# wfus/Fully-Homomorphic-Image-Processing

Measured on AMD Instinct MI355X. Metric: encrypted 8x8 blocks/sec (homomorphic DCT+quant), higher is better.
Workload: dtype f64

## Files before the change

### fully-homomorphic-image-processing_amd/csrc/dct_fused.hip

```cpp
#include "internal.h"

#include <cstdlib>

#include "fp64_core.h"

#pragma clang fp contract(off)

namespace {
using namespace fp64;

template <int L, int LE> struct Shape {
    static constexpr int N = 1 << L, E = 1 << LE, TP = N >> LE, NP = (L + LE - 1) / LE, LDS_WORDS = N + (N >> LE);
};
__host__ __device__ constexpr int g_lo(int L, int LE, int p) { return (L - LE * p - LE) < 0 ? 0 : (L - LE * p - LE); }
__host__ __device__ constexpr int g_stages(int L, int LE, int p) { return (L - LE * p) > LE ? LE : (L - LE * p); }
template <int LO, int LE> __device__ __forceinline__ int g_index(int tid, int r) {
    return ((tid >> LO) << (LO + LE)) | (r << LO) | (tid & ((1 << LO) - 1));
}
template <int LO, int LE> __device__ __forceinline__ int g_pad(int j) { return j + ((j >> (LO + LE)) << LO); }

template <int L, int LE, int P> struct PassTw {
    static constexpr int LO = g_lo(L, LE, P), S = g_stages(L, LE, P), NTW = (1 << LE) - 1;
    static constexpr int rb(int u) { return (L - 1 - (LE * P + u)) - LO; }
    static constexpr int count(int u) { return 1 << (LE - 1 - rb(u)); }
// ... 70 lines not shown
            for (int b0 = 0; b0 < E / 2; b0 += KB) {
                double t[KB * M], wm[KB * M];
#pragma unroll
                for (int kb = 0; kb < KB; kb++) {
                    const int b = b0 + kb, r0 = ((b >> rb) << (rb + 1)) | (b & ((1 << rb) - 1)), r1 = r0 | (1 << rb);
                    const double wv = w[T::offset(u) + (r0 >> (rb + 1))];
#pragma unroll
                    for (int m = 0; m < M; m++) {
                        const double X = x[m][r0], Y = x[m][r1];
                        x[m][r0] = X + Y;
                        t[kb * M + m] = X - Y; wm[kb * M + m] = wv;
                    }
                }
                mmv<KB * M>(t, wm, p, pinv);
#pragma unroll
                for (int kb = 0; kb < KB; kb++) {
                    const int b = b0 + kb, r0 = ((b >> rb) << (rb + 1)) | (b & ((1 << rb) - 1)), r1 = r0 | (1 << rb);
#pragma unroll
                    for (int m = 0; m < M; m++) x[m][r1] = t[kb * M + m];
                }
            }
        }
    }
}

template <int L, int LE, int LO_FROM, int LO_TO, int M>
__device__ __forceinline__ void transpose(double (&x)[M][1 << LE], double *lds, int tid, int &phase) {
    constexpr int PL = imin(LO_FROM, LO_TO), E = 1 << LE;
    constexpr bool WAVE_LOCAL = (Shape<L, LE>::TP <= 64) || (LO_FROM <= 6 && LO_TO <= 6);
#pragma unroll
    for (int m = 0; m < M; m++) {
        double *buf = lds + (phase & 1) * Shape<L, LE>::LDS_WORDS;
        phase++;
#pragma unroll
        for (int r = 0; r < E; r++) buf[g_pad<PL, LE>(g_index<LO_FROM, LE>(tid, r))] = x[m][r];
        if constexpr (WAVE_LOCAL) {
            __builtin_amdgcn_fence(__ATOMIC_RELEASE, "wavefront");
            __builtin_amdgcn_wave_barrier();
            __builtin_amdgcn_fence(__ATOMIC_ACQUIRE, "wavefront");
        } else {
            __syncthreads();
        }
#pragma unroll
        for (int r = 0; r < E; r++) x[m][r] = buf[g_pad<PL, LE>(g_index<LO_TO, LE>(tid, r))];
    }
}

template <int L, int LE, int M, typename PRE, int P = 0>
__device__ __forceinline__ void ntt_fwd(double (&x)[M][1 << LE], double (&w)[(1 << LE) - 1], const double *__restrict__ tw, double p, double pinv,
                                        double *lds, int tid, int &phase, PRE pre) {
    if constexpr (P + 1 < Shape<L, LE>::NP) {
        double wn[(1 << LE) - 1];
        if (LE >= 4) load_tw<L, LE, P + 1>(wn, tw, tid);
        fwd_pass<L, LE, P, M>(x, w, p, pinv);
        if (LE < 4) load_tw<L, LE, P + 1>(wn, tw, tid);
        if constexpr (P + 2 == Shape<L, LE>::NP) pre();
        transpose<L, LE, g_lo(L, LE, P), g_lo(L, LE, P + 1), M>(x, lds, tid, phase);
        ntt_fwd<L, LE, M, PRE, P + 1>(x, wn, tw, p, pinv, lds, tid, phase, pre);
    } else {
        fwd_pass<L, LE, P, M>(x, w, p, pinv);
    }
}
template <int L, int LE, int M, bool BIG, int P = Shape<L, LE>::NP - 1>
__device__ __forceinline__ void ntt_inv(double (&x)[M][1 << LE], double (&w)[(1 << LE) - 1], const double *__restrict__ itw, double p, double pinv,
                                        double *lds, int tid, int &phase) {
    if constexpr (P > 0) {
        double wn[(1 << LE) - 1];
        if (LE >= 4) load_tw<L, LE, P - 1>(wn, itw, tid);
        inv_pass<L, LE, P, M>(x, w, 0.0, p, pinv);
        if (LE < 4) load_tw<L, LE, P - 1>(wn, itw, tid);
        if constexpr (BIG) {
#pragma unroll
            for (int m = 0; m < M; m++)
#pragma unroll
                for (int r = 0; r < (1 << LE); r++) x[m][r] = red(x[m][r], p, pinv);
        }
        transpose<L, LE, g_lo(L, LE, P), g_lo(L, LE, P - 1), M>(x, lds, tid, phase);
        ntt_inv<L, LE, M, BIG, P - 1>(x, wn, itw, p, pinv, lds, tid, phase);
    } else {
        inv_pass<L, LE, P, M>(x, w, itw[0], p, pinv);
    }
}

constexpr double PACK_BIAS = 6755399441055744.0;
template <int E, int TP>
__device__ __forceinline__ void store_packed(char *__restrict__ ob, u32 vo, u32 so, const double (&x)[E]) {
    static_assert(E == 8, "packed layout is defined for 8 values per thread");
    u32 lo[8], hi[8];
#pragma unroll
    for (int r = 0; r < 8; r++) {
        const double t = x[r] + PACK_BIAS;
        lo[r] = (u32)__double2loint(t);
        hi[r] = (u32)__double2hiint(t);
    }
#pragma unroll
    for (int q = 0; q < 4; q++) *(u64 *)(ob + (size_t)(so + q * TP * 8) + vo) = (u64)lo[2 * q] | ((u64)lo[2 * q + 1] << 32);
    u32 h[2];
#pragma unroll
    for (int g = 0; g < 2; g++) {
        const u32 p01 = __builtin_amdgcn_perm(hi[4 * g + 1], hi[4 * g + 0], 0x0c0c0400u);
        const u32 p23 = __builtin_amdgcn_perm(hi[4 * g + 3], hi[4 * g + 2], 0x0c0c0400u);
        h[g] = __builtin_amdgcn_perm(p23, p01, 0x05040100u);
    }
    *(u64 *)(ob + (size_t)(so + 4 * TP * 8) + vo) = (u64)h[0] | ((u64)h[1] << 32);
}
typedef __attribute__((address_space(3))) void lc_lptr;
template <int NT>
__device__ __forceinline__ void stage_consts(gwin_t w, u32 voff, u32 soff, u32 cstride_bytes, double *stg) {
#pragma unroll
    for (int i0 = 0; i0 < NT; i0 += 2) {
        const int i = (i0 + 1 < NT) ? i0 : NT - 2;
        __builtin_amdgcn_raw_ptr_buffer_load_lds(w, (lc_lptr *)(stg + i * 64), 16, voff, soff + (u32)i * cstride_bytes, 0, 0);
    }
}

template <int L, int LE, bool BIG, int HALF, bool PACK, bool LDSC>
__device__ __forceinline__ void rows_body(const u64 *__restrict__ in, double *__restrict__ mid, const double *__restrict__ consts,
                                          const double *__restrict__ tw, const Work &wk, double p, double pinv, u32 k, double *lds) {
    using SH = Shape<L, LE>;
    constexpr int N = SH::N, TP = SH::TP, E = SH::E, NC = HalfC<HALF>::NC, FIRST = HalfC<HALF>::FIRST;
    const int tid = threadIdx.x;
    const size_t poly_words = (size_t)k * N, ct_words = 2 * poly_words;
    const size_t base = ((size_t)wk.blk * 64 + 8 * wk.line) * ct_words + (size_t)wk.poly * poly_words + (size_t)wk.prime * N;
    const gwin_t win_in = gwin(in + base), win_mid = gwin(mid + base);
    const u32 vo = (u32)tid * 8u, ctb = (u32)(ct_words * 8);
    double w0[E - 1];
    load_tw<L, LE, 0>(w0, tw, tid);
    double x[4][E];
    u64 ra[2][E], rb[2][E];
    auto issue = [&](int m) {
#pragma unroll
        for (int r = 0; r < E; r++) {
            ra[m & 1][r] = gld_u64(win_in, vo, (u32)m * ctb + r * TP * 8);
            rb[m & 1][r] = gld_u64(win_in, vo, (u32)(7 - m) * ctb + r * TP * 8);
        }
    };
    auto combine = [&](int m) {
#pragma unroll
        for (int r = 0; r < E; r++) {
            const u64 A = ra[m & 1][r], B = rb[m & 1][r];
            x[m][r] = HALF ? u52_biased(A) - u52_biased(B) : u52_to_f64(A + B);
        }
    };
    if constexpr (LE >= 4) {
        issue(0);
        issue(1);
        asm volatile("" ::: "memory");
        combine(0);
        issue(2);
        asm volatile("" ::: "memory");
        combine(1);
        issue(3);
        asm volatile("" ::: "memory");
        combine(2);
        combine(3);
    } else {
#pragma unroll
        for (int m = 0; m < 4; m++) {
            issue(m);
            combine(m);
            asm volatile("" ::: "memory");
        }
    }
    const size_t cstride = (size_t)k * N;
    const gwin_t win_c = gwin(consts + (size_t)FIRST * cstride + (size_t)wk.prime * N);
    const u32 csb = (u32)(cstride * 8);
    double cn[9];
    auto fetch = [&](int r) {
#pragma unroll
        for (int i = 0; i < NC; i++) cn[i] = gld_f64(win_c, vo, (u32)i * csb + r * TP * 8);
    };
    int phase = 0;
    ntt_fwd<L, LE, 4>(x, w0, tw, p, pinv, lds, tid, phase, [&] { if (LE >= 4) fetch(0); });
    const int lane = tid & 63;
    double *stg = lds + (tid >> 6) * (2 * NC * 64);
    const u32 svoff = (u32)(((size_t)(lane >> 5) * cstride + (tid & ~63) + 2 * (lane & 31)) * sizeof(double));
    constexpr int NDMA = (NC + 1) / 2;
    if constexpr (LDSC) {
        __builtin_amdgcn_sched_barrier(0);
        __syncthreads();
        stage_consts<NC>(win_c, svoff, 0, csb, stg);
    }
#pragma unroll
    for (int r = 0; r < E; r++) {
        double c[9];
        if constexpr (LDSC) {
            if (r + 1 < E) stage_consts<NC>(win_c, svoff, (r + 1) * TP * 8, csb, stg + ((r + 1) & 1) * NC * 64);
            if (r + 1 < E) asm volatile("s_waitcnt vmcnt(%0)" ::"n"(NDMA) : "memory");
            else asm volatile("s_waitcnt vmcnt(0)" ::: "memory");
            const double *sr = stg + (r & 1) * NC * 64 + lane;
#pragma unroll
            for (int i = 0; i < NC; i++) c[i] = sr[i * 64];
        } else {
        if (LE < 4) fetch(r);
#pragma unroll
        for (int i = 0; i < NC; i++) c[i] = cn[i];
        if (LE >= 4 && r + 1 < E) fetch(r + 1);
        }
        line_half<HALF>(x[0][r], x[1][r], x[2][r], x[3][r], c, p, pinv);
        if (BIG) {
#pragma unroll
            for (int m = 0; m < 4; m++) x[m][r] = red(x[m][r], p, pinv);
        } else if (PACK && HALF == 0) {
            x[0][r] = red(x[0][r], p, pinv);
            x[2][r] = red(x[2][r], p, pinv);
        }
        if constexpr (LDSC) asm volatile("" ::"v"(x[0][r]), "v"(x[1][r]), "v"(x[2][r]), "v"(x[3][r]) : "memory");
    }
#pragma unroll
    for (int m = 0; m < 4; m++) {
        const u32 so = (u32)(2 * m + HALF) * ctb;
        if constexpr (PACK) {
            store_packed<E, TP>((char *)(mid + base), vo, so, x[m]);
        } else {
#pragma unroll
            for (int r = 0; r < E; r++) gst_f64(win_mid, vo, so + r * TP * 8, x[m][r]);
        }
    }
}

__host__ __device__ constexpr int occ_waves(int tp, int lds_words) {
    return ((2 * lds_words * 16 <= 160 * 1024) ? 2 : 1) * tp / 256 < 1 ? 1 : ((2 * lds_words * 16 <= 160 * 1024) ? 2 : 1) * tp / 256;
}
template <int L, int LE> struct Occ { static constexpr int W = occ_waves(Shape<L, LE>::TP, Shape<L, LE>::LDS_WORDS); };

template <int L, int LE, bool BIG, bool PACK, bool LDSC>
__global__ __launch_bounds__((Shape<L, LE>::TP), (Occ<L, LE>::W)) void k_dct_rows(const u64 *__restrict__ in, double *__restrict__ mid,
                                                                  const double *__restrict__ consts, const double *__restrict__ tw_all,
                                                                  const Modulus *__restrict__ mods, u32 k) {
    __shared__ double lds[2 * Shape<L, LE>::LDS_WORDS];
    const Work wk = decode(blockIdx.x, k);
    const double p = (double)mods[wk.prime].q, pinv = 1.0 / p;
    const double *tw = tw_all + (size_t)wk.prime * Shape<L, LE>::N;
    if (wk.half) rows_body<L, LE, BIG, 1, PACK, LDSC>(in, mid, consts, tw, wk, p, pinv, k, lds);
    else rows_body<L, LE, BIG, 0, PACK, LDSC>(in, mid, consts, tw, wk, p, pinv, k, lds);
}

template <int L, int LE, bool BIG, int HALF, bool PACK>
__device__ __forceinline__ void cols_body(const double *__restrict__ mid, u64 *__restrict__ out, const double *__restrict__ consts,
                                          const double *__restrict__ itw, const Work &wk, double p, double pinv, u32 k, double *lds) {
    using SH = Shape<L, LE>;
    constexpr int N = SH::N, TP = SH::TP, E = SH::E, NC = HalfC<HALF>::NC, FIRST = HalfC<HALF>::FIRST;
    constexpr int LASTP = SH::NP - 1;
    const int tid = threadIdx.x;
    const size_t poly_words = (size_t)k * N, ct_words = 2 * poly_words;
    const size_t base = ((size_t)wk.blk * 64 + wk.line) * ct_words + (size_t)wk.poly * poly_words + (size_t)wk.prime * N;
    const size_t cstride = (size_t)k * N;
    const gwin_t win_mid = gwin(mid + base), win_out = gwin(out + base);
    const gwin_t win_c = gwin(consts + (size_t)FIRST * cstride + (size_t)wk.prime * N);
    const gwin_t win_s = gwin(consts + (size_t)(12 + 8 * HALF + wk.line) * cstride + (size_t)wk.prime * N);
    const u32 vo = (u32)tid * 8u, rsb = (u32)(ct_words * 64), csb = (u32)(cstride * 8);
    const double pbias = p + 4503599627370496.0;
    double cn[9], sn[4];
    auto fetch = [&](int r) {
#pragma unroll
        for (int i = 0; i < NC; i++) cn[i] = gld_f64(win_c, vo, (u32)i * csb + r * TP * 8);
#pragma unroll
        for (int m = 0; m < 4; m++) sn[m] = gld_f64(win_s, vo, (u32)(16 * m) * csb + r * TP * 8);
    };
    double wl[E - 1];
    if constexpr (!PACK) {
        fetch(0);
        load_tw<L, LE, LASTP>(wl, itw, tid);
    }
    double x[4][E];
    if constexpr (PACK) {
        u64 wa[4][5], wb[4][5];
#pragma unroll
        for (int m = 0; m < 4; m++) {
#pragma unroll
            for (int q = 0; q < 5; q++) {
                wa[m][q] = gld_u64(win_mid, vo, (u32)m * rsb + q * TP * 8);
                wb[m][q] = gld_u64(win_mid, vo, (u32)(7 - m) * rsb + q * TP * 8);
            }
        }
#pragma unroll
        for (int m = 0; m < 4; m++) {
#pragma unroll
            for (int r = 0; r < E; r++) {
                const u32 la = (r & 1) ? (u32)(wa[m][r >> 1] >> 32) : (u32)wa[m][r >> 1];
                const u32 lb = (r & 1) ? (u32)(wb[m][r >> 1] >> 32) : (u32)wb[m][r >> 1];
                const u32 hwa = (r & 4) ? (u32)(wa[m][4] >> 32) : (u32)wa[m][4], hwb = (r & 4) ? (u32)(wb[m][4] >> 32) : (u32)wb[m][4];
                const double ta = __hiloint2double((int)(0x43380000u + (u32)(int)(signed char)(hwa >> (8 * (r & 3)))), (int)la);
                const double tb = __hiloint2double((int)(0x43380000u + (u32)(int)(signed char)(hwb >> (8 * (r & 3)))), (int)lb);
                x[m][r] = HALF ? ta - tb : ta + (tb - 2.0 * PACK_BIAS);
            }
        }
    } else {
#pragma unroll
        for (int m = 0; m < 4; m++) {
#pragma unroll
            for (int r = 0; r < E; r++) {
                const double A = gld_f64(win_mid, vo, (u32)m * rsb + r * TP * 8), B = gld_f64(win_mid, vo, (u32)(7 - m) * rsb + r * TP * 8);
                x[m][r] = HALF ? A - B : A + B;
            }
        }
    }
    if constexpr (PACK) load_tw<L, LE, LASTP>(wl, itw, tid);
#pragma unroll
    for (int r = 0; r < E; r++) {
        double c[9], sc[4];
        if (PACK) fetch(r);
#pragma unroll
        for (int i = 0; i < NC; i++) c[i] = cn[i];
#pragma unroll
        for (int m = 0; m < 4; m++) sc[m] = sn[m];
        if (!PACK && r + 1 < E) fetch(r + 1);
        line_half<HALF>(x[0][r], x[1][r], x[2][r], x[3][r], c, p, pinv);
        double y[4] = {x[0][r], x[1][r], x[2][r], x[3][r]};
        mmv<4>(y, sc, p, pinv);
#pragma unroll
        for (int m = 0; m < 4; m++) x[m][r] = y[m];
    }
    int phase = 0;
    ntt_inv<L, LE, 4, BIG>(x, wl, itw, p, pinv, lds, tid, phase);
#pragma unroll
    for (int m = 0; m < 4; m++) {
#pragma unroll
        for (int r = 0; r < E; r++) gst_u64(win_out, vo, (u32)(2 * m + HALF) * rsb + r * TP * 8, f64_to_residue(x[m][r], pbias));
    }
}

template <int L, int LE, bool BIG, bool PACK>
__global__ __launch_bounds__((Shape<L, LE>::TP), (Occ<L, LE>::W)) void k_dct_cols(const double *__restrict__ mid, u64 *__restrict__ out,
                                                                  const double *__restrict__ consts, const double *__restrict__ itw_all,
                                                                  const Modulus *__restrict__ mods, u32 k) {
    __shared__ double lds[2 * Shape<L, LE>::LDS_WORDS];
    const Work wk = decode(blockIdx.x, k);
    const double p = (double)mods[wk.prime].q, pinv = 1.0 / p;
    const double *itw = itw_all + (size_t)wk.prime * Shape<L, LE>::N;
    if (wk.half) cols_body<L, LE, BIG, 1, PACK>(mid, out, consts, itw, wk, p, pinv, k, lds);
    else cols_body<L, LE, BIG, 0, PACK>(mid, out, consts, itw, wk, p, pinv, k, lds);
}

template <int L, int LE>
__global__ __launch_bounds__((Shape<L, LE>::TP), (Occ<L, LE>::W)) void k_dct_one_launch(const u64 *__restrict__ in, double *__restrict__ mid, u64 *__restrict__ out,
                                                                        const double *__restrict__ consts, const double *__restrict__ tw_all,
                                                                        const double *__restrict__ itw_all, const Modulus *__restrict__ mods, u32 k,
                                                                        u32 n_blocks, u32 dist, u32 *__restrict__ arrived, u32 *__restrict__ err) {
    __shared__ double lds[2 * Shape<L, LE>::LDS_WORDS];
    const u32 xcd = blockIdx.x & 7, seq = blockIdx.x >> 3, chunk = seq >> 5, r = seq & 31;
    const bool is_row = r < 16;
    const long j = is_row ? (long)chunk : (long)chunk - (long)(dist & 0xffffu);
    const u32 n_units = n_blocks * 2 * k;
    if (j < 0) return;
    const u64 g = (u64)j * 8 + xcd;
    if (g >= n_units) return;
    Work wk;
    wk.prime = (u32)(g / (n_blocks * 2));
    const u32 rem = (u32)(g - (u64)wk.prime * n_blocks * 2);
    wk.blk = rem >> 1;
    wk.poly = rem & 1;
    wk.line = (r & 15) >> 1;
    wk.half = r & 1;
    const double p = (double)mods[wk.prime].q, pinv = 1.0 / p;
    if (is_row) {
        const double *tw = tw_all + (size_t)wk.prime * Shape<L, LE>::N;
        if (wk.half) rows_body<L, LE, false, 1, true, true>(in, mid, consts, tw, wk, p, pinv, k, lds);
        else rows_body<L, LE, false, 0, true, true>(in, mid, consts, tw, wk, p, pinv, k, lds);
        if (dist & 0x10000u) return;
        __syncthreads();
        if (threadIdx.x == 0) {
            __threadfence();
            atomicAdd(arrived + g, 1u);
        }
    } else {
        if (!(dist & 0x10000u) && threadIdx.x == 0) {
            u32 spins = 0;
            while (__hip_atomic_load(arrived + g, __ATOMIC_RELAXED, __HIP_MEMORY_SCOPE_AGENT) < 16u) {
                __builtin_amdgcn_s_sleep(8);
                if (++spins > (1u << 24)) { atomicExch(err, 1u); break; }
            }
            __threadfence();
        }
        __syncthreads();
        const double *itw = itw_all + (size_t)wk.prime * Shape<L, LE>::N;
        if (wk.half) cols_body<L, LE, false, 1, true>(mid, out, consts, itw, wk, p, pinv, k, lds);
        else cols_body<L, LE, false, 0, true>(mid, out, consts, itw, wk, p, pinv, k, lds);
    }
}

__global__ void k_consts_to_f64(const ulonglong2 *__restrict__ in, double *__restrict__ out, const Modulus *__restrict__ mods, u32 k, u32 n, u32 le, u32 total) {
    const u32 i = blockIdx.x * blockDim.x + threadIdx.x;
    if (i >= total) return;
    const u32 pos = i % n, rowbase = i - pos;
    const u32 tp = n >> le, r = pos / tp, t = pos % tp;
    const u32 j = (t << le) + r;
    const u32 src = (j & 15) * (n >> 4) + (j >> 4);
    const u64 q = mods[(i / n) % k].q;
    const u64 w = in[rowbase + src].x;
    out[i] = w > q / 2 ? -(double)(q - w) : (double)w;
}

template <int L, int LE>
__global__ __launch_bounds__((Shape<L, LE>::TP), (Occ<L, LE>::W)) void k_rgb2ycc_f64(u64 *__restrict__ R, u64 *__restrict__ G, u64 *__restrict__ Bc,
                                                                     const double *__restrict__ consts, const double *__restrict__ tw_all,
                                                                     const double *__restrict__ itw_all, const Modulus *__restrict__ mods,
                                                                     const u64 *__restrict__ yoff, u32 yoff_len, u32 k, u32 group, u64 gstride) {
    using SH = Shape<L, LE>;
    constexpr int N = SH::N, TP = SH::TP, E = SH::E, LASTP = SH::NP - 1;
    __shared__ double lds[2 * SH::LDS_WORDS];
    const int tid = threadIdx.x;
    const u32 per_prime = gridDim.x / k;
    const u32 prime = blockIdx.x / per_prime;
    const u32 pp = blockIdx.x - prime * per_prime;
    const u32 poly = pp & 1, pix = pp >> 1;
    const u64 q = mods[prime].q;
    const double p = (double)q, pinv = 1.0 / p;
    const double *tw = tw_all + (size_t)prime * N, *itw = itw_all + (size_t)prime * N;
    const size_t pix_off = group ? (size_t)(pix / group) * gstride + (size_t)(pix % group) * 2 * k * N : (size_t)pix * 2 * k * N;
    const size_t off = pix_off + ((size_t)poly * k + prime) * N + tid;
    double w0[E - 1];
    load_tw<L, LE, 0>(w0, tw, tid);
    double x[3][E];
    {
        const u64 *src[3] = {R + off, G + off, Bc + off};
#pragma unroll
        for (int m = 0; m < 3; m++)
#pragma unroll
            for (int r = 0; r < E; r++) x[m][r] = u52_to_f64(src[m][r * TP]);
    }
    int phase = 0;
    ntt_fwd<L, LE, 3>(x, w0, tw, p, pinv, lds, tid, phase, [] {});
    double wl[E - 1];
    load_tw<L, LE, LASTP>(wl, itw, tid);
    const double *cp = consts + (size_t)prime * N + tid;
    const size_t cstride = (size_t)k * N;
#pragma unroll
    for (int r = 0; r < E; r++) {
        double c[9], y[9];
#pragma unroll
        for (int i = 0; i < 9; i++) { c[i] = cp[(size_t)i * cstride + r * TP]; y[i] = x[i % 3][r]; }
        mmv<9>(y, c, p, pinv);
        x[0][r] = y[0] + y[1] + y[2];
        x[1][r] = y[3] - y[4] + y[5];
        x[2][r] = y[6] - y[7] - y[8];
    }
    ntt_inv<L, LE, 3, false>(x, wl, itw, p, pinv, lds, tid, phase);
    u64 *dst[3] = {R + off, G + off, Bc + off};
#pragma unroll
    for (int m = 0; m < 3; m++)
#pragma unroll
        for (int r = 0; r < E; r++) {
            double v = x[m][r];
            v = v < 0.0 ? v + p : v;
            u64 o = f64_to_u52(v);
            if (m == 0 && poly == 0) {
                const u32 j = (u32)(r * TP + tid);
                if (j < yoff_len) o = submod(o, yoff[(size_t)prime * yoff_len + j], q);
            }
            dst[m][r * TP] = o;
        }
}

template <int L, int LE, int M, int MODE>
__global__ __launch_bounds__((Shape<L, LE>::TP), (Occ<L, LE>::W)) void k_poly_f64(const u64 *__restrict__ in, u64 *__restrict__ out,
                                                                  const ulonglong2 *__restrict__ plain, const double *__restrict__ tw_all,
                                                                  const double *__restrict__ itw_all, const Modulus *__restrict__ mods, u32 k) {
    using SH = Shape<L, LE>;
    constexpr int N = SH::N, TP = SH::TP, E = SH::E, LASTP = SH::NP - 1;
    static_assert(LE == 3, "slot-order mapping below is written for 8 values per thread");
// ... 17 lines not shown
            for (int r = 0; r < E; r++) x[m][r] = u52_to_f64(src[r * TP]);
        }
        ntt_fwd<L, LE, M>(x, w0, tw, p, pinv, lds, tid, phase, [] {});
    } else {
#pragma unroll
        for (int m = 0; m < M; m++) {
            const u64 *src = in + ((size_t)(g * M + m) * k + prime) * N + slot0;
#pragma unroll
            for (int r = 0; r < E; r++) x[m][r] = u52_to_f64(src[r * (N >> 4)]);
        }
    }
    if constexpr (MODE == 0) {
#pragma unroll
        for (int m = 0; m < M; m++) {
            u64 *dst = out + ((size_t)(g * M + m) * k + prime) * N + slot0;
#pragma unroll
            for (int r = 0; r < E; r++) {
                double v = red(x[m][r], p, pinv);
                v = v < 0.0 ? v + p : v;
                dst[r * (N >> 4)] = f64_to_u52(v);
            }
        }
        return;
    }
    double wl[E - 1];
    load_tw<L, LE, LASTP>(wl, itw, tid);
    if constexpr (MODE == 2) {
        const ulonglong2 *pp = plain + (size_t)prime * N + slot0;
#pragma unroll
        for (int r = 0; r < E; r++) {
            const double w = u52_to_f64(pp[r * (N >> 4)].x);
            double y[M], wm[M];
#pragma unroll
            for (int m = 0; m < M; m++) { y[m] = x[m][r]; wm[m] = w; }
            mmv<M>(y, wm, p, pinv);
#pragma unroll
            for (int m = 0; m < M; m++) x[m][r] = y[m];
        }
    }
    ntt_inv<L, LE, M, false>(x, wl, itw, p, pinv, lds, tid, phase);
#pragma unroll
    for (int m = 0; m < M; m++) {
        u64 *dst = out + ((size_t)(g * M + m) * k + prime) * N + tid;
#pragma unroll
        for (int r = 0; r < E; r++) {
            double v = x[m][r];
            v = v < 0.0 ? v + p : v;
            dst[r * TP] = f64_to_u52(v);
        }
    }
}

}


static u32 dct_shape_le(const fhe_ctx *c) {
    if (c->opt.dct_le != 3) return 4;
    if (c->logn == 12 && c->max_prime_bits <= 40) return 3;
    if (c->logn == 13 || c->logn == 11) return 3;
    return 4;
}

bool fhe_dct_f64_supported(const fhe_ctx *c) {
    return c && c->qb.d_tw_f64 && c->max_prime_bits <= 47 && (c->logn >= 10 && c->logn <= 13);
}

int fhe_dct_f64_make_consts(const fhe_ctx *c, fhe_dct_plan *plan, hipStream_t st) {
    const u32 total = DCT_NCONST * c->k * c->n;
    HIP_TRY(hipMalloc(&plan->d_consts_f64, sizeof(double) * total));
    const u32 le = dct_shape_le(c);
    k_consts_to_f64<<<(total + 255) / 256, 256, 0, st>>>(plan->d_consts, plan->d_consts_f64, c->qb.d_mod, c->k, c->n, le, total);
    KERNEL_CHECK();
    return FHE_OK;
}



template <int L, int LE>
static void launch_pair(const fhe_ctx *c, const fhe_dct_plan *plan, const u64 *in, u64 *out, double *mid, unsigned grid, bool big, hipStream_t st, int which) {
    constexpr int TP = Shape<L, LE>::TP;
    if constexpr (LE == 4) {
        if (big) {
            if (which & 1) k_dct_rows<L, LE, true, false, false><<<grid, TP, 0, st>>>(in, mid, plan->d_consts_f64, c->qb.d_tw_f64, c->qb.d_mod, c->k);
            if (which & 2) k_dct_cols<L, LE, true, false><<<grid, TP, 0, st>>>(mid, out, plan->d_consts_f64, c->qb.d_itw_f64, c->qb.d_mod, c->k);
            return;
        }
    }
    if constexpr (LE == 3) {
        if (big) {
            if (which & 1) k_dct_rows<L, LE, true, false, false><<<grid, TP, 0, st>>>(in, mid, plan->d_consts_f64, c->qb.d_tw_f64, c->qb.d_mod, c->k);
            if (which & 2) k_dct_cols<L, LE, true, false><<<grid, TP, 0, st>>>(mid, out, plan->d_consts_f64, c->qb.d_itw_f64, c->qb.d_mod, c->k);
            return;
        }
        if (c->max_prime_bits <= 37 && c->opt.dct_pack) {
            if (which & 1) {
                if (c->opt.dct_ldsc) k_dct_rows<L, LE, false, true, true><<<grid, TP, 0, st>>>(in, mid, plan->d_consts_f64, c->qb.d_tw_f64, c->qb.d_mod, c->k);
                else k_dct_rows<L, LE, false, true, false><<<grid, TP, 0, st>>>(in, mid, plan->d_consts_f64, c->qb.d_tw_f64, c->qb.d_mod, c->k);
            }
            if (which & 2) k_dct_cols<L, LE, false, true><<<grid, TP, 0, st>>>(mid, out, plan->d_consts_f64, c->qb.d_itw_f64, c->qb.d_mod, c->k);
            return;
        }
    }
    {
        if (which & 1) k_dct_rows<L, LE, false, false, false><<<grid, TP, 0, st>>>(in, mid, plan->d_consts_f64, c->qb.d_tw_f64, c->qb.d_mod, c->k);
        if (which & 2) k_dct_cols<L, LE, false, false><<<grid, TP, 0, st>>>(mid, out, plan->d_consts_f64, c->qb.d_itw_f64, c->qb.d_mod, c->k);
    }
}

int fhe_dct_f64_launch(const fhe_ctx *c, const fhe_dct_plan *plan, const u64 *in, u64 *out, u64 n_blocks, double *mid, hipStream_t st, int which) {
    const u64 items = n_blocks * 8 * 2 * c->k;
    const u64 grid = items * 2;
    if (grid > 0x7fffffffULL) return fail(FHE_ERR_PARAM, "too many blocks for one launch");
    if ((u64)c->k * c->n >= (1ULL << 21)) return fail(FHE_ERR_PARAM, "fused FP64 path: a block of ciphertexts exceeds the 2 GiB addressing window");
    const bool big = c->max_prime_bits > 40;
    if (c->opt.dct_one_launch && which == 3 && c->logn == 12 && dct_shape_le(c) == 3 && c->max_prime_bits <= 37 && c->opt.dct_pack && c->d_arrived) {
        const u64 n_units = n_blocks * 2 * c->k;
        if (n_units > c->arrived_cap) return fail(FHE_ERR_PARAM, "one-launch experiment: wave too large for the arrival counters");
        HIP_TRY(hipMemsetAsync(c->d_arrived, 0, (n_units + 1) * sizeof(u32), st));
        const u32 dist = c->opt.dct_one_launch;
        const u64 chunks = (n_units + 7) / 8 + (dist & 0xffffu);
        k_dct_one_launch<12, 3><<<(unsigned)(chunks * 32 * 8), Shape<12, 3>::TP, 0, st>>>(in, mid, out, plan->d_consts_f64, c->qb.d_tw_f64, c->qb.d_itw_f64, c->qb.d_mod,
                                                                                       c->k, (u32)n_blocks, dist, c->d_arrived + 1, c->d_arrived);
        KERNEL_CHECK();
        u32 timed_out = 0;
        HIP_TRY(hipMemcpyAsync(&timed_out, c->d_arrived, sizeof(u32), hipMemcpyDeviceToHost, st));
        HIP_TRY(hipStreamSynchronize(st));
        if (timed_out) return fail(FHE_ERR_HIP, "one-launch experiment: a column workgroup timed out waiting for its row transforms; the output is incomplete");
        return FHE_OK;
    }
    switch (c->logn) {
        case 10: launch_pair<10, 4>(c, plan, in, out, mid, (unsigned)grid, big, st, which); break;
        case 11: launch_pair<11, 3>(c, plan, in, out, mid, (unsigned)grid, big, st, which); break;
        case 12: if (dct_shape_le(c) == 3) launch_pair<12, 3>(c, plan, in, out, mid, (unsigned)grid, false, st, which); else launch_pair<12, 4>(c, plan, in, out, mid, (unsigned)grid, big, st, which); break;
        case 13: if (dct_shape_le(c) == 3) launch_pair<13, 3>(c, plan, in, out, mid, (unsigned)grid, big, st, which); else launch_pair<13, 4>(c, plan, in, out, mid, (unsigned)grid, big, st, which); break;
        default: return fail(FHE_ERR_PARAM, "fused FP64 path supports n in {1024, 2048, 4096, 8192}");
    }
    KERNEL_CHECK();
    return FHE_OK;
}

bool fhe_rgb_f64_supported(const fhe_ctx *c) {
    return fhe_dct_f64_supported(c) && c->logn == 12 && c->max_prime_bits <= 40;
}

int fhe_rgb_f64_make_consts(const fhe_ctx *c, const ulonglong2 *d_c, double **out, hipStream_t st) {
    const u32 total = 9 * c->k * c->n;
    HIP_TRY(hipMalloc(out, sizeof(double) * total));
    k_consts_to_f64<<<(total + 255) / 256, 256, 0, st>>>(d_c, *out, c->qb.d_mod, c->k, c->n, 3, total);
    KERNEL_CHECK();
    return FHE_OK;
}

int fhe_rgb_f64_launch(const fhe_ctx *c, u64 *r, u64 *g, u64 *b, u64 count, const double *consts, const u64 *yoff, u32 yoff_len, hipStream_t st, u32 group, u64 gstride) {
    const u64 grid = count * 2 * c->k;
    if (grid > 0x7fffffffULL) return fail(FHE_ERR_PARAM, "too many pixels for one launch");
    k_rgb2ycc_f64<12, 3><<<(unsigned)grid, Shape<12, 3>::TP, 0, st>>>(r, g, b, consts, c->qb.d_tw_f64, c->qb.d_itw_f64, c->qb.d_mod, yoff, yoff_len, c->k, group, gstride);
    KERNEL_CHECK();
    return FHE_OK;
}

int fhe_poly_f64_launch(int mode, const fhe_ctx *c, const u64 *in, u64 *out, u64 n_polys, const ulonglong2 *plain, hipStream_t st) {
    const u64 grid2 = (n_polys / 2) * c->k, grid1 = n_polys * c->k;
    if (grid1 > 0x7fffffffULL) return fail(FHE_ERR_PARAM, "too many polynomials for one launch");
    constexpr int TP = Shape<12, 3>::TP;
#define LAUNCH_POLY(M, GRID)                                                                                                          \
    switch (mode) {                                                                                                                   \
        case 0: k_poly_f64<12, 3, M, 0><<<(unsigned)(GRID), TP, 0, st>>>(in, out, plain, c->qb.d_tw_f64, c->qb.d_itw_f64, c->qb.d_mod, c->k); break; \
        case 1: k_poly_f64<12, 3, M, 1><<<(unsigned)(GRID), TP, 0, st>>>(in, out, plain, c->qb.d_tw_f64, c->qb.d_itw_f64, c->qb.d_mod, c->k); break; \
        default: k_poly_f64<12, 3, M, 2><<<(unsigned)(GRID), TP, 0, st>>>(in, out, plain, c->qb.d_tw_f64, c->qb.d_itw_f64, c->qb.d_mod, c->k); break; \
    }
    if (n_polys % 2 == 0) { LAUNCH_POLY(2, grid2) } else { LAUNCH_POLY(1, grid1) }
#undef LAUNCH_POLY
    KERNEL_CHECK();
    return FHE_OK;
}

namespace {
using namespace fp64;

template <int HALF>
__device__ __forceinline__ void idct_half(double (&v)[4], const double (&c)[12], double p, double pinv) {
    if constexpr (HALF == 0) {
        double y[3] = {v[1] + v[3], v[3], v[1]};
        const double w[3] = {c[0], c[2], c[1]};
        mmv<3>(y, w, p, pinv);
        const double t2 = y[0] + y[1], t3 = y[0] + y[2], t0 = v[0] + v[2], t1 = v[0] - v[2];
        v[0] = t0 + t3;
        v[1] = t1 + t2;
// ... 161 lines not shown
```

### fully-homomorphic-image-processing_amd/csrc/fhe_hip.hip

```cpp
#include "internal.h"

#include <cmath>
#include <cstdarg>
#include <cstdio>
#include <cstdlib>
#include <cstring>
#include <algorithm>
#include <condition_variable>
#include <mutex>
#include <string>
#include <vector>

#include "host_math.h"

static thread_local std::string g_err;
int fhe_fail(int code, const char *fmt, ...) {
    char buf[512];
    va_list ap;
    va_start(ap, fmt);
    vsnprintf(buf, sizeof buf, fmt, ap);
    va_end(ap);
    g_err = buf;
    return code;
}
// ... 113 lines not shown
    }
    return FHE_OK;
}
void fhe_free_base(BaseTables &B) {
    if (B.d_tw) (void)hipFree(B.d_tw);
    if (B.d_itw) (void)hipFree(B.d_itw);
    if (B.d_mod) (void)hipFree(B.d_mod);
    if (B.d_tw_f64) (void)hipFree(B.d_tw_f64);
    if (B.d_itw_f64) (void)hipFree(B.d_itw_f64);
    if (B.d_tw_pm) (void)hipFree(B.d_tw_pm);
    if (B.d_itw_pm) (void)hipFree(B.d_itw_pm);
    if (B.d_pm) (void)hipFree(B.d_pm);
    if (B.d_tw_pm3) (void)hipFree(B.d_tw_pm3);
    if (B.d_itw_pm3) (void)hipFree(B.d_itw_pm3);
    B.d_tw_pm = B.d_itw_pm = B.d_tw_pm3 = B.d_itw_pm3 = nullptr;
    B.d_pm = nullptr;
    B.pm_class = 0;
    B.d_tw_f64 = B.d_itw_f64 = nullptr;
    B.d_tw = B.d_itw = nullptr;
    B.d_mod = nullptr;
}

static bool env_on(const char *name) { const char *e = getenv(name); return e && *e && !(e[0] == '0' && !e[1]); }

extern "C" int fhe_default_coeff_modulus(uint32_t n, int preset, uint64_t *q_out) {
    static const u64 s3_4096[] = {0xffffee001ULL, 0xffffc4001ULL, 0x1ffffe0001ULL};
    static const u64 s3_8192[] = {0x7fffffd8001ULL, 0x7fffffc8001ULL, 0xfffffffc001ULL, 0xffffff6c001ULL, 0xfffffebc001ULL};
    static const u64 s23_2048[] = {0x3fffffff000001ULL};
    static const u64 s23_4096[] = {0x7fffffff380001ULL, 0x3fffffff000001ULL};
    static const u64 s23_8192[] = {0x7fffffff380001ULL, 0x7ffffffef00001ULL, 0x3fffffff000001ULL, 0x3ffffffef40001ULL};
    static const u64 s23_16384[] = {0x7fffffff380001ULL, 0x7ffffffef00001ULL, 0x7ffffffeac0001ULL, 0x7ffffffe700001ULL, 0x7ffffffe600001ULL, 0x7ffffffe4c0001ULL,
                                    0x3fffffff000001ULL, 0x3ffffffef40001ULL};
    const u64 *src = nullptr;
    int cnt = 0;
#define PICK(a) do { src = a; cnt = (int)(sizeof(a) / sizeof(a[0])); } while (0)
    if (preset == 0) {
        if (n == 4096) PICK(s3_4096);
        else if (n == 8192) PICK(s3_8192);
        else if (n == 2048 || n == 1024) PICK(s23_2048);
        else if (n == 16384) PICK(s23_16384);
    } else if (preset == 1) {
        if (n == 2048 || n == 1024) PICK(s23_2048);
        else if (n == 4096) PICK(s23_4096);
        else if (n == 8192) PICK(s23_8192);
        else if (n == 16384) PICK(s23_16384);
    }
#undef PICK
    if (!src) return fail(FHE_ERR_PARAM, "no default coefficient modulus for n=%u preset=%d", n, preset);
    for (int i = 0; i < cnt; ++i) q_out[i] = src[i];
    return cnt;
}

extern "C" int fhe_ctx_create(uint32_t n, const uint64_t *q, uint32_t k, uint64_t t, int device, fhe_ctx **out) {
    using namespace hostmath;
    if (!out || !q) return fail(FHE_ERR_PARAM, "null argument");
    *out = nullptr;
    if (k == 0 || k > FHE_MAX_K) return fail(FHE_ERR_PARAM, "coeff modulus count %u out of range", k);
    if (n < 1024 || n > 16384 || (n & (n - 1))) return fail(FHE_ERR_PARAM, "poly_modulus_degree %u unsupported", n);
    if (t < 2) return fail(FHE_ERR_PARAM, "plain modulus too small");
    int ndev = 0;
    if (hipGetDeviceCount(&ndev) != hipSuccess || ndev <= 0)
        return fail(FHE_ERR_HIP, "no HIP device available (this library has no CPU fallback)");
    if (device < 0 || device >= ndev) return fail(FHE_ERR_PARAM, "device %d out of range", device);
    HIP_TRY(hipSetDevice(device));
    std::vector<u64> primes(k);
    for (u32 i = 0; i < k; ++i) primes[i] = q[i];
    for (u32 i = 0; i < k; ++i) {
        if (primes[i] >> 61) return fail(FHE_ERR_PARAM, "modulus %u exceeds 61 bits", i);
        if (!is_prime(primes[i]) || (primes[i] - 1) % (2ULL * n)) return fail(FHE_ERR_PARAM, "modulus %u is not an NTT prime for n=%u", i, n);
        if (t >= primes[i]) return fail(FHE_ERR_PARAM, "plain modulus must be below every coefficient modulus");
        for (u32 j = 0; j < i; ++j)
            if (primes[j] == primes[i]) return fail(FHE_ERR_PARAM, "duplicate modulus");
    }
    fhe_ctx *c = new fhe_ctx();
    {
        FheOptions &o = c->opt;
        auto off = [](const char *name) { const char *e = getenv(name); return e && e[0] == '0' && !e[1]; };
        o.force_u64 = env_on("FHE_DCT_FORCE_U64");
        o.dct_pipeline = env_on("FHE_DCT_PIPELINE");
        if (const char *e = getenv("FHE_DCT_WAVE_BLOCKS")) { const u64 v = strtoull(e, nullptr, 10); if (v) o.dct_wave_blocks = v; }
        if (const char *e = getenv("FHE_DCT_LE")) o.dct_le = atoi(e) == 4 ? 4 : 3;
        o.dct_pack = !off("FHE_DCT_PACK");
        o.dct_ldsc = !off("FHE_DCT_LDSC");
        o.dct_u64_fused = !off("FHE_DCT_U64_FUSED");
        if (const char *e = getenv("FHE_DCT_ONE_LAUNCH")) o.dct_one_launch = (u32)atoi(e);
        o.relin_fused = env_on("FHE_RELIN_FUSED");
        o.filter_xcd = !off("FHE_FILTER_XCD");
        o.galois_staged = env_on("FHE_GALOIS_STAGED");
        o.galois_gather_lds = env_on("FHE_GALOIS_GATHER_LDS");
        o.relin_steps = env_on("FHE_RELIN_STEPS");
        o.enc_unfused = env_on("FHE_ENC_UNFUSED");
        { const char *e = std::getenv("FHE_ENC_OCC"); o.enc_occ4 = e && e[0] == '4'; }
        o.ntt_nolazy = env_on("FHE_NTT_NOLAZY");
        o.ntt_single = env_on("FHE_NTT_SINGLE");
        o.ntt_nopm = env_on("FHE_NTT_NOPM");
        o.behz_aux61 = env_on("FHE_BEHZ_AUX61");
        o.behz_chunk3 = env_on("FHE_BEHZ_CHUNK3");
        o.behz_tensor_canon = env_on("FHE_BEHZ_TENSOR_CANON");
        o.behz_tensor_single = env_on("FHE_BEHZ_TENSOR_SINGLE");
        o.behz_fused_prepare = env_on("FHE_BEHZ_FUSED_PREPARE");
        o.cubic_unfused = env_on("FHE_CUBIC_UNFUSED");
        o.plain_sum_unfused = env_on("FHE_PLAIN_SUM_UNFUSED");
        o.behz_square_full = env_on("FHE_BEHZ_SQUARE_FULL");
    }
    c->n = n;
    c->k = k;
    c->t = t;
    c->device = device;
    while ((1u << c->logn) < n) ++c->logn;
    for (u32 i = 0; i < k; ++i) c->max_prime_bits = std::max(c->max_prime_bits, bit_length(primes[i]));
    int rc = fhe_build_base(c->qb, primes, n, c->logn, c->max_prime_bits <= 47);
    if (rc) { delete c; return rc; }
    BigUInt Q(1);
    for (u32 i = 0; i < k; ++i) Q.mul_small(primes[i]);
    const u64 q_mod_t = Q.mod_small(t);
    c->upper_half_threshold = (t + 1) >> 1;
    for (u32 i = 0; i < k; ++i) {
        const u64 qi = primes[i];
        c->plain_upper_half_increment[i] = submod(0, t % qi, qi);
        c->upper_half_increment[i] = q_mod_t % qi;
        c->delta_mod[i] = mulmod(submod(0, q_mod_t % qi, qi), invmod(t % qi, qi), qi);
    }
    if (env_on("FHE_BEHZ_EAGER") && (rc = fhe_behz_ensure(c))) { fhe_ctx_destroy(c); return rc; }
    if (c->opt.dct_one_launch) {
        c->arrived_cap = 1024 * 2 * (u64)k;
        if (hipMalloc((void **)&c->d_arrived, (c->arrived_cap + 1) * sizeof(u32)) != hipSuccess) { fhe_ctx_destroy(c); return fail(FHE_ERR_HIP, "arrival counters"); }
    }
    bool ok = !c->opt.dct_pipeline || hipStreamCreateWithFlags(&c->aux_stream, hipStreamNonBlocking) == hipSuccess;
    for (int i = 0; i < 2 && ok && c->opt.dct_pipeline; ++i)
        ok = hipEventCreateWithFlags(&c->ev_rows[i], hipEventDisableTiming) == hipSuccess &&
             hipEventCreateWithFlags(&c->ev_cols[i], hipEventDisableTiming) == hipSuccess;
    if (!ok) { fhe_ctx_destroy(c); return fail(FHE_ERR_HIP, "stream/event creation failed"); }
    *out = c;
    return FHE_OK;
}

extern "C" int fhe_ctx_destroy(fhe_ctx *c) {
    if (!c) return FHE_OK;
    if (c->aux_stream) (void)hipStreamDestroy(c->aux_stream);
    if (c->d_arrived) (void)hipFree(c->d_arrived);
    for (int i = 0; i < 2; ++i) {
        if (c->ev_rows[i]) (void)hipEventDestroy(c->ev_rows[i]);
        if (c->ev_cols[i]) (void)hipEventDestroy(c->ev_cols[i]);
    }
    for (fhe_ctx::RgbConsts *r : c->rgb) {
        if (r->d_c) (void)hipFree(r->d_c);
        if (r->d_c_f64) (void)hipFree(r->d_c_f64);
        if (r->d_off) (void)hipFree(r->d_off);
        delete r;
    }
    for (fhe_ctx::RgbConsts *r : c->ycc) {
        if (r->d_c) (void)hipFree(r->d_c);
        if (r->d_off) (void)hipFree(r->d_off);
        delete r;
    }
    fhe_behz_free(c);
    fhe_free_base(c->qb);
    delete c;
    return FHE_OK;
}
extern "C" int fhe_ctx_device(const fhe_ctx *c) { return c ? c->device : -1; }
extern "C" int fhe_ctx_bind_thread(const fhe_ctx *c) {
    if (!c) return fail(FHE_ERR_PARAM, "null argument");
    HIP_TRY(hipSetDevice(c->device));
    return FHE_OK;
}
// ... 1409 lines not shown
```

### fully-homomorphic-image-processing_amd/csrc/internal.h

```cpp
#pragma once
#include "../../include/fhe_hip.h"

#include <hip/hip_runtime.h>

#include <mutex>
#include <string>
#include <vector>

#include "modarith.h"
#include "ntt_core.h"

int fhe_fail(int code, const char *fmt, ...) __attribute__((format(printf, 2, 3)));
#define fail fhe_fail
#define HIP_TRY(expr)                                                                             \
    do {                                                                                          \
        hipError_t e_ = (expr);                                                                   \
        if (e_ != hipSuccess) return fail(FHE_ERR_HIP, "%s: %s", #expr, hipGetErrorString(e_));   \
    } while (0)
#define KERNEL_CHECK()                                                                            \
    do {                                                                                          \
        hipError_t e_ = hipGetLastError();                                                        \
        if (e_ != hipSuccess) return fail(FHE_ERR_HIP, "kernel launch: %s", hipGetErrorString(e_)); \
    } while (0)

struct BaseTables {
    std::vector<u64> primes;
    ulonglong2 *d_tw = nullptr, *d_itw = nullptr;
    Modulus *d_mod = nullptr;
    std::vector<Modulus> h_mod;
    double *d_tw_f64 = nullptr, *d_itw_f64 = nullptr;
    ulonglong2 *d_tw_pm = nullptr, *d_itw_pm = nullptr;
    ulonglong2 *d_tw_pm3 = nullptr, *d_itw_pm3 = nullptr;
    PmMod *d_pm = nullptr;
    int pm_class = 0;
    RnsBase dev() const { return RnsBase{d_tw, d_itw, d_mod, (u32)primes.size(), d_tw_pm, d_itw_pm, d_pm}; }
};

struct FheOptions {
    bool force_u64 = false;
    bool dct_pipeline = false;
    u64 dct_wave_blocks = 256;
    int dct_le = 3;
    bool dct_pack = true;
    bool dct_ldsc = true;
    bool dct_u64_fused = true;
    u32 dct_one_launch = 0;
    bool ntt_nolazy = false;
    bool ntt_single = false;
    bool ntt_nopm = false;
    bool behz_aux61 = false;
    bool behz_chunk3 = false;
    bool behz_tensor_canon = false;
    bool behz_tensor_single = false;
    bool behz_square_full = false;
    bool plain_sum_unfused = false;
    bool cubic_unfused = false;
    bool enc_unfused = false;
    bool enc_occ4 = false;
    bool relin_steps = false;
    bool relin_fused = false;
    bool filter_xcd = true;
    bool galois_staged = false;
    bool galois_gather_lds = false;
    bool behz_fused_prepare = false;
};

struct fhe_ctx {
    u32 n = 0, logn = 0, k = 0;
    FheOptions opt;
    u64 t = 0;
    int device = 0;
    int max_prime_bits = 0;
    BaseTables qb;
    u64 upper_half_threshold = 0;
    u64 plain_upper_half_increment[FHE_MAX_K] = {0};
    u64 delta_mod[FHE_MAX_K] = {0};
    u64 upper_half_increment[FHE_MAX_K] = {0};
    struct BehzTables *behz = nullptr;
    mutable std::once_flag behz_once;
    int behz_rc = 0;
    std::string behz_err;
    u32 *d_arrived = nullptr;
    u64 arrived_cap = 0;
    hipStream_t aux_stream = nullptr;
    hipEvent_t ev_rows[2] = {nullptr, nullptr}, ev_cols[2] = {nullptr, nullptr};
    struct RgbConsts {
        int int_coeffs = -1, frac_coeffs = -1;
        ulonglong2 *d_c = nullptr;
        double *d_c_f64 = nullptr;
        u64 *d_off = nullptr;
        u32 off_len = 0;
    };
    mutable std::vector<RgbConsts *> rgb;
    mutable std::vector<RgbConsts *> ycc;
    mutable std::mutex rgb_mutex;
};

#define DCT_NCONST 76
extern const double kDctConst[12];
struct fhe_dct_plan {
    ulonglong2 *d_consts = nullptr;
    double *d_consts_f64 = nullptr;
    ulonglong2 *d_consts_le3 = nullptr;
    u32 k = 0, n = 0;
    bool has_quant = false;
};

inline float fhe_resize_ref_coord(u32 i, u32 dst_len, u32 src_len) { return (float)((float)i / (float)(dst_len - 1) * (float)src_len - 0.5); }

#define DISPATCH_L(logn, ...)                                                    \
    switch (logn) {                                                              \
        case 10: { constexpr int L = 10; __VA_ARGS__; } break;                   \
        case 11: { constexpr int L = 11; __VA_ARGS__; } break;                   \
        case 12: { constexpr int L = 12; __VA_ARGS__; } break;                   \
        case 13: { constexpr int L = 13; __VA_ARGS__; } break;                   \
        case 14: { constexpr int L = 14; __VA_ARGS__; } break;                   \
        default: return fail(FHE_ERR_PARAM, "unsupported log2(n)=%u", logn);     \
    }

struct CMap {
    const u32 *idx;
    u64 div, cnt, off;
    __device__ __forceinline__ u64 operator()(u64 c) const { return idx ? idx[c] : (cnt ? ((off + c / div) % cnt) : c); }
};

#define FHE_PLAIN_SUM_MAX_TERMS 16
struct PlainSumTerms {
// ... 41 lines not shown
```

Measured before the change: 85480.

## Stage column-pass DCT constants through LDS with double-buffered prefetch

Adds an LDSC variant of the column kernel for the packed LE=3 path. Per-row DCT constants, and the scale constants on one half, are loaded asynchronously into a double-buffered LDS staging area with explicit vmcnt waits, instead of being fetched into registers per thread. The goal is to cut redundant global loads and register pressure by reusing the rows-kernel staging scheme. It also rewrites the packed high-byte sign-extension as a single v_perm with a changed PACK_BIAS, which trims ALU work during unpacking. The path is on by default behind an env flag, and the exact hand-tuned waitcnt counts put correctness at risk.

```diff
diff --git a/fully-homomorphic-image-processing_amd/csrc/dct_fused.hip b/fully-homomorphic-image-processing_amd/csrc/dct_fused.hip
--- a/fully-homomorphic-image-processing_amd/csrc/dct_fused.hip
+++ b/fully-homomorphic-image-processing_amd/csrc/dct_fused.hip
@@ -176,7 +176,7 @@
     }
 }
 
-constexpr double PACK_BIAS = 6755399441055744.0;
+constexpr double PACK_BIAS = 6755949196869632.0;
 template <int E, int TP>
 __device__ __forceinline__ void store_packed(char *__restrict__ ob, u32 vo, u32 so, const double (&x)[E]) {
     static_assert(E == 8, "packed layout is defined for 8 values per thread");
@@ -330,7 +330,7 @@
     else rows_body<L, LE, BIG, 0, PACK, LDSC>(in, mid, consts, tw, wk, p, pinv, k, lds);
 }
 
-template <int L, int LE, bool BIG, int HALF, bool PACK>
+template <int L, int LE, bool BIG, int HALF, bool PACK, bool LDSC>
 __device__ __forceinline__ void cols_body(const double *__restrict__ mid, u64 *__restrict__ out, const double *__restrict__ consts,
                                           const double *__restrict__ itw, const Work &wk, double p, double pinv, u32 k, double *lds) {
     using SH = Shape<L, LE>;
@@ -375,8 +375,9 @@
                 const u32 la = (r & 1) ? (u32)(wa[m][r >> 1] >> 32) : (u32)wa[m][r >> 1];
                 const u32 lb = (r & 1) ? (u32)(wb[m][r >> 1] >> 32) : (u32)wb[m][r >> 1];
                 const u32 hwa = (r & 4) ? (u32)(wa[m][4] >> 32) : (u32)wa[m][4], hwb = (r & 4) ? (u32)(wb[m][4] >> 32) : (u32)wb[m][4];
-                const double ta = __hiloint2double((int)(0x43380000u + (u32)(int)(signed char)(hwa >> (8 * (r & 3)))), (int)la);
-                const double tb = __hiloint2double((int)(0x43380000u + (u32)(int)(signed char)(hwb >> (8 * (r & 3)))), (int)lb);
+                const u32 sel = 0x03020104u + (u32)(r & 3);
+                const double ta = __hiloint2double((int)__builtin_amdgcn_perm(hwa, 0x43380000u, sel), (int)la);
+                const double tb = __hiloint2double((int)__builtin_amdgcn_perm(hwb, 0x43380000u, sel), (int)lb);
                 x[m][r] = HALF ? ta - tb : ta + (tb - 2.0 * PACK_BIAS);
             }
         }
@@ -391,6 +392,53 @@
         }
     }
     if constexpr (PACK) load_tw<L, LE, LASTP>(wl, itw, tid);
+    if constexpr (LDSC) {
+        static_assert(PACK && LE == 3, "LDS staging of the column constants is built for the packed LE = 3 path");
+        static_assert(2 * 9 * 64 * (TP / 64) <= 2 * SH::LDS_WORDS, "staging regions exceed the exchange buffers");
+        constexpr bool SLDS = HALF == 0;
+        constexpr int NREG = NC + (SLDS ? 4 : 0);
+        constexpr int NDMA = (NC + 1) / 2 + (SLDS ? 2 : 0);
+        constexpr int NSREG = SLDS ? 0 : 4;
+#pragma unroll
+        for (int m = 0; m < 4; m++)
+            asm volatile("" ::"v"(x[m][0]), "v"(x[m][1]), "v"(x[m][2]), "v"(x[m][3]), "v"(x[m][4]), "v"(x[m][5]), "v"(x[m][6]), "v"(x[m][7]));
+        const int lane = tid & 63;
+        double *stg = lds + __builtin_amdgcn_readfirstlane(tid >> 6) * (2 * 9 * 64);
+        const u32 lvo = (u32)(((tid & ~63) + 2 * (lane & 31)) * sizeof(double));
+        const u32 svoff = lvo + (u32)(lane >> 5) * csb, ssvoff = lvo + (u32)(lane >> 5) * 16u * csb;
+        auto stage = [&](int r) {
+            double *reg = stg + (r & 1) * NREG * 64;
+            stage_consts<NC>(win_c, svoff, r * TP * 8, csb, reg);
+            if constexpr (SLDS) stage_consts<4>(win_s, ssvoff, r * TP * 8, 16u * csb, reg + NC * 64);
+        };
+        stage(0);
+#pragma unroll
+        for (int r = 0; r < E; r++) {
+            double c[9], sc[4];
+            if constexpr (!SLDS) {
+#pragma unroll
+                for (int m = 0; m < 4; m++) sc[m] = gld_f64(win_s, vo, (u32)(16 * m) * csb + r * TP * 8);
+            }
+            if (r + 1 < E) stage(r + 1);
+            if (r + 1 < E) asm volatile("s_waitcnt vmcnt(%0)" ::"n"(NDMA + NSREG) : "memory");
+            else asm volatile("s_waitcnt vmcnt(%0)" ::"n"(NSREG) : "memory");
+            const double *sr = stg + (r & 1) * NREG * 64 + lane;
+#pragma unroll
+            for (int i = 0; i < NC; i++) c[i] = sr[i * 64];
+            if constexpr (SLDS) {
+#pragma unroll
+                for (int m = 0; m < 4; m++) sc[m] = sr[(NC + m) * 64];
+            }
+            line_half<HALF>(x[0][r], x[1][r], x[2][r], x[3][r], c, p, pinv);
+            double y[4] = {x[0][r], x[1][r], x[2][r], x[3][r]};
+            mmv<4>(y, sc, p, pinv);
+#pragma unroll
+            for (int m = 0; m < 4; m++) x[m][r] = y[m];
+            asm volatile("" ::"v"(x[0][r]), "v"(x[1][r]), "v"(x[2][r]), "v"(x[3][r]) : "memory");
+        }
+        __builtin_amdgcn_sched_barrier(0);
+        __syncthreads();
+    } else {
 #pragma unroll
     for (int r = 0; r < E; r++) {
         double c[9], sc[4];
@@ -406,6 +454,7 @@
 #pragma unroll
         for (int m = 0; m < 4; m++) x[m][r] = y[m];
     }
+    }
     int phase = 0;
     ntt_inv<L, LE, 4, BIG>(x, wl, itw, p, pinv, lds, tid, phase);
 #pragma unroll
@@ -415,7 +464,7 @@
     }
 }
 
-template <int L, int LE, bool BIG, bool PACK>
+template <int L, int LE, bool BIG, bool PACK, bool LDSC>
 __global__ __launch_bounds__((Shape<L, LE>::TP), (Occ<L, LE>::W)) void k_dct_cols(const double *__restrict__ mid, u64 *__restrict__ out,
                                                                   const double *__restrict__ consts, const double *__restrict__ itw_all,
                                                                   const Modulus *__restrict__ mods, u32 k) {
@@ -423,8 +472,8 @@
     const Work wk = decode(blockIdx.x, k);
     const double p = (double)mods[wk.prime].q, pinv = 1.0 / p;
     const double *itw = itw_all + (size_t)wk.prime * Shape<L, LE>::N;
-    if (wk.half) cols_body<L, LE, BIG, 1, PACK>(mid, out, consts, itw, wk, p, pinv, k, lds);
-    else cols_body<L, LE, BIG, 0, PACK>(mid, out, consts, itw, wk, p, pinv, k, lds);
+    if (wk.half) cols_body<L, LE, BIG, 1, PACK, LDSC>(mid, out, consts, itw, wk, p, pinv, k, lds);
+    else cols_body<L, LE, BIG, 0, PACK, LDSC>(mid, out, consts, itw, wk, p, pinv, k, lds);
 }
 
 template <int L, int LE>
@@ -469,8 +518,8 @@
         }
         __syncthreads();
         const double *itw = itw_all + (size_t)wk.prime * Shape<L, LE>::N;
-        if (wk.half) cols_body<L, LE, false, 1, true>(mid, out, consts, itw, wk, p, pinv, k, lds);
-        else cols_body<L, LE, false, 0, true>(mid, out, consts, itw, wk, p, pinv, k, lds);
+        if (wk.half) cols_body<L, LE, false, 1, true, false>(mid, out, consts, itw, wk, p, pinv, k, lds);
+        else cols_body<L, LE, false, 0, true, false>(mid, out, consts, itw, wk, p, pinv, k, lds);
     }
 }
 
@@ -654,14 +703,14 @@
     if constexpr (LE == 4) {
         if (big) {
             if (which & 1) k_dct_rows<L, LE, true, false, false><<<grid, TP, 0, st>>>(in, mid, plan->d_consts_f64, c->qb.d_tw_f64, c->qb.d_mod, c->k);
-            if (which & 2) k_dct_cols<L, LE, true, false><<<grid, TP, 0, st>>>(mid, out, plan->d_consts_f64, c->qb.d_itw_f64, c->qb.d_mod, c->k);
+            if (which & 2) k_dct_cols<L, LE, true, false, false><<<grid, TP, 0, st>>>(mid, out, plan->d_consts_f64, c->qb.d_itw_f64, c->qb.d_mod, c->k);
             return;
         }
     }
     if constexpr (LE == 3) {
         if (big) {
             if (which & 1) k_dct_rows<L, LE, true, false, false><<<grid, TP, 0, st>>>(in, mid, plan->d_consts_f64, c->qb.d_tw_f64, c->qb.d_mod, c->k);
-            if (which & 2) k_dct_cols<L, LE, true, false><<<grid, TP, 0, st>>>(mid, out, plan->d_consts_f64, c->qb.d_itw_f64, c->qb.d_mod, c->k);
+            if (which & 2) k_dct_cols<L, LE, true, false, false><<<grid, TP, 0, st>>>(mid, out, plan->d_consts_f64, c->qb.d_itw_f64, c->qb.d_mod, c->k);
             return;
         }
         if (c->max_prime_bits <= 37 && c->opt.dct_pack) {
@@ -669,13 +718,16 @@
                 if (c->opt.dct_ldsc) k_dct_rows<L, LE, false, true, true><<<grid, TP, 0, st>>>(in, mid, plan->d_consts_f64, c->qb.d_tw_f64, c->qb.d_mod, c->k);
                 else k_dct_rows<L, LE, false, true, false><<<grid, TP, 0, st>>>(in, mid, plan->d_consts_f64, c->qb.d_tw_f64, c->qb.d_mod, c->k);
             }
-            if (which & 2) k_dct_cols<L, LE, false, true><<<grid, TP, 0, st>>>(mid, out, plan->d_consts_f64, c->qb.d_itw_f64, c->qb.d_mod, c->k);
+            if (which & 2) {
+                if (c->opt.dct_ldsc_cols) k_dct_cols<L, LE, false, true, true><<<grid, TP, 0, st>>>(mid, out, plan->d_consts_f64, c->qb.d_itw_f64, c->qb.d_mod, c->k);
+                else k_dct_cols<L, LE, false, true, false><<<grid, TP, 0, st>>>(mid, out, plan->d_consts_f64, c->qb.d_itw_f64, c->qb.d_mod, c->k);
+            }
             return;
         }
     }
     {
         if (which & 1) k_dct_rows<L, LE, false, false, false><<<grid, TP, 0, st>>>(in, mid, plan->d_consts_f64, c->qb.d_tw_f64, c->qb.d_mod, c->k);
-        if (which & 2) k_dct_cols<L, LE, false, false><<<grid, TP, 0, st>>>(mid, out, plan->d_consts_f64, c->qb.d_itw_f64, c->qb.d_mod, c->k);
+        if (which & 2) k_dct_cols<L, LE, false, false, false><<<grid, TP, 0, st>>>(mid, out, plan->d_consts_f64, c->qb.d_itw_f64, c->qb.d_mod, c->k);
     }
 }
 
diff --git a/fully-homomorphic-image-processing_amd/csrc/fhe_hip.hip b/fully-homomorphic-image-processing_amd/csrc/fhe_hip.hip
--- a/fully-homomorphic-image-processing_amd/csrc/fhe_hip.hip
+++ b/fully-homomorphic-image-processing_amd/csrc/fhe_hip.hip
@@ -219,6 +219,7 @@
         if (const char *e = getenv("FHE_DCT_LE")) o.dct_le = atoi(e) == 4 ? 4 : 3;
         o.dct_pack = !off("FHE_DCT_PACK");
         o.dct_ldsc = !off("FHE_DCT_LDSC");
+        o.dct_ldsc_cols = !off("FHE_DCT_LDSC_COLS");
         o.dct_u64_fused = !off("FHE_DCT_U64_FUSED");
         if (const char *e = getenv("FHE_DCT_ONE_LAUNCH")) o.dct_one_launch = (u32)atoi(e);
         o.relin_fused = env_on("FHE_RELIN_FUSED");
diff --git a/fully-homomorphic-image-processing_amd/csrc/internal.h b/fully-homomorphic-image-processing_amd/csrc/internal.h
--- a/fully-homomorphic-image-processing_amd/csrc/internal.h
+++ b/fully-homomorphic-image-processing_amd/csrc/internal.h
@@ -43,6 +43,7 @@
     int dct_le = 3;
     bool dct_pack = true;
     bool dct_ldsc = true;
+    bool dct_ldsc_cols = true;
     bool dct_u64_fused = true;
     u32 dct_one_launch = 0;
     bool ntt_nolazy = false;
```

Result: no change. 85270 (-0.2%).
